# choyingw/SynergyNet

Hardware: NVIDIA H100
Metric: faces/sec (120x120, batch 1024 per GPU, backbone + 3DMM params + 68 landmarks) (higher is better)
Workload: dtype f32

## Files before the change

### synergynet_b200/csrc/kernels_fused.cuh

```cuda
#pragma once
#include "common.cuh"
#include "tc_common.cuh"

namespace syn {

constexpr int kFusedWorkerWarps = 8;
static_assert(kFusedWorkerWarps % 4 == 0, "worker warps form whole warpgroups");

__host__ __device__ constexpr int ceil_div_c(int a, int b) { return (a + b - 1) / b; }
__host__ __device__ constexpr int round_up_c(int a, int b) { return ceil_div_c(a, b) * b; }

template <int CIN_, int CHID_, int NC_, int COUT_, int W_, int STRIDE_, int RO_, int FACES_, bool RES_, int WSTREAM_>
struct FusedCfg {
  static constexpr bool RES = RES_;
  static constexpr bool WSTREAM = WSTREAM_ > 0;
  static constexpr int CIN = CIN_;
  static constexpr int CIN_P = round_up_c(CIN_, 16);
  static constexpr int CHID = CHID_, NC = NC_, NCHUNK = CHID_ / NC_;
  static constexpr int COUT = COUT_, COUT_P = round_up_c(COUT_, 16);
  static constexpr int W = W_, STRIDE = STRIDE_, WO = (W_ - 1) / STRIDE_ + 1;
  static constexpr int RO = RO_, STRIPS = WO / RO_, FACES = FACES_;
  static constexpr int RWIN = (RO_ - 1) * STRIDE_ + 3;
  static constexpr int ROWS_MAX = (RWIN < W_ ? RWIN : W_);
  static constexpr int M1_MAX = FACES_ * ROWS_MAX * W_;
// ... 41 lines not shown
  int* sat;
  int npass;
#ifdef SYN_FUSED_TRACE
  int trace_id;
#endif
};

#ifdef SYN_FUSED_TRACE
__device__ long long g_fused_trace[18 * 2 * 64 * 8];
#define SYN_TRACE(role, chunk, ev)                                                                        \
  do {                                                                                                    \
    if (trace_on) g_fused_trace[((p.trace_id * 2 + (role)) * 64 + (chunk)) * 8 + (ev)] = clock64();      \
  } while (0)
#else
#define SYN_TRACE(role, chunk, ev) do { } while (0)
#endif

template <int THREADS>
__device__ __forceinline__ void group_bar_sync(int grp) {
  switch (grp) {
    case 0: asm volatile("bar.sync 1, %0;" ::"n"(THREADS) : "memory"); break;
    case 1: asm volatile("bar.sync 2, %0;" ::"n"(THREADS) : "memory"); break;
    case 2: asm volatile("bar.sync 3, %0;" ::"n"(THREADS) : "memory"); break;
    default: asm volatile("bar.sync 4, %0;" ::"n"(THREADS) : "memory"); break;
  }
}

__host__ __device__ constexpr int fused_d2_pieces(int cout_p, int slabs, int nwg) {
  int s = 1;
  while (slabs * s < nwg && (cout_p / (2 * s)) % 8 == 0) s *= 2;
  return s;
}

template <int N, int KSTEPS, int NPASS>
__device__ __forceinline__ void fused_mma_group(float* acc, uint32_t d_hi, uint32_t a_lo, uint32_t a_plane, uint32_t a_kstep,
                                                uint32_t b_lo, uint32_t b_plane, uint32_t b_kstep, bool acc_in) {
  tc::wgmma_fence();
#pragma unroll
  for (int pass = 0; pass < NPASS; ++pass)
#pragma unroll
    for (int ks = 0; ks < KSTEPS; ++ks)
      tc::wgmma_f16<N>(acc, tc::desc64(d_hi, a_lo + (((pass == 2 ? a_plane : 0) + ks * a_kstep) >> 4)),
                       tc::desc64(d_hi, b_lo + (((pass == 1 ? b_plane : 0) + ks * b_kstep) >> 4)),
                       (acc_in || pass > 0 || ks > 0) ? 1u : 0u);
  tc::wgmma_commit();
}

template <class C>
__global__ void __launch_bounds__((kFusedWorkerWarps + 1) * 32, 1) fused_mbconv_kernel(const FusedArgs p) {
  constexpr int NWW = kFusedWorkerWarps;
  constexpr int NWT = NWW * 32;
  constexpr int NWG = NWW / 4;
  constexpr int NKG_ = C::NC / 8;
  constexpr int NG = 1;
  constexpr int WPG = NWW / NG, TPG = WPG * 32;
  constexpr int KPG = NKG_ / NG;
  constexpr int NSPL = fused_d2_pieces(C::COUT_P, C::SLABS2, NWG);
  constexpr int N2 = C::COUT_P / NSPL;
  constexpr int IPW = ceil_div_c(C::SLABS2 * NSPL, NWG);
  static_assert(N2 % 8 == 0 && N2 <= 256, "MMA N");
  using namespace tc;
  extern __shared__ __align__(1024) uint8_t smem_raw[];
  __shared__ __align__(8) uint64_t bar_w, bar_wfull[4], bar_wempty[4];

  uint8_t* smem = smem_raw + ((1024u - (smem_u32(smem_raw) & 1023u)) & 1023u);
  const int tid = threadIdx.x, warp = tid >> 5;
// ... 196 lines not shown
        SYN_TRACE(0, c, 3);
      };
      {
        SYN_TRACE(0, 0, 0);
        const uint8_t* w0 = chunk_slot(g, 0);
        group_bar_sync<TPG>(grp);
        SYN_TRACE(0, 0, 1);
        if constexpr (C::STRIPS > 1) {
          constexpr int CQ = KPG * 2;
          if (iy0 < 0)
            for (int i = gtid; i < C::HS_COLS * CQ; i += TPG)
              *reinterpret_cast<float4*>(sH + (size_t)(i / CQ) * C::HS_STRIDE + grp * KPG * 8 + (i % CQ) * 4) =
                  make_float4(0.f, 0.f, 0.f, 0.f);
          if (iy0 + C::RWIN - 1 > C::W - 1)
            for (int i = gtid; i < C::HS_COLS * CQ; i += TPG)
              *reinterpret_cast<float4*>(sH + (size_t)((C::RWIN - 1) * C::HS_COLS + i / CQ) * C::HS_STRIDE +
                                         grp * KPG * 8 + (i % CQ) * 4) = make_float4(0.f, 0.f, 0.f, 0.f);
        }
        issue_g1(wg < slabs1, acc1[0], wg, w0);
        gemm1_epi1(0, w0);
      }
      for (int c = 0; c < C::NCHUNK; ++c, ++g) {
        const int slot = C::WSTREAM ? (int)(g % C::WSTAGES) : c;
        const uint8_t* wch = sWch + slot * C::CHUNK_BYTES;
        const float* dwc = reinterpret_cast<const float*>(wch + C::CH_DW);
        group_bar_sync<TPG>(grp);
        SYN_TRACE(0, c, 4);
        const bool more = c + 1 < C::NCHUNK;
        const uint8_t* wn = wch;
        if constexpr (!LATE_G1) {
          if (more) wn = chunk_slot(g + 1, c + 1);
          issue_g1(more && wg < slabs1, acc1[0], wg, wn);
        }
        if constexpr (C::STRIDE == 1 && ((C::WO >= 15 && C::WO <= 30) || C::WO == 8)) {
          constexpr int XL = (C::WO >= 15) ? 8 : 4, YL = 8 / XL;
          constexpr int CPR = (C::WO + 1) / 2, XG2 = (CPR + XL - 1) / XL, RP2 = (C::RO + 1) / 2;
          constexpr int RPU = (RP2 + YL - 1) / YL, UPK = RPU * XG2;
          const int l8 = tid & 7, qh = (tid >> 3) & 1;
          const int lx = l8 % XL, ly = l8 / XL;
          const bool mir = (l8 & 4) != 0;
          const int units = KPG * nfaces * UPK;
          for (int u = gtid >> 4; u < units; u += TPG / 16) {
            const int kgl = u / (nfaces * UPK), r1 = u - kgl * (nfaces * UPK);
            const int f = r1 / UPK, r2 = r1 - f * UPK;
            const int rpu = r2 / XG2, xg = r2 - rpu * XG2;
            const int kg = grp * KPG + kgl, j0 = kg * 8 + qh * 4;
            const int ox = 2 * (xg * XL + lx), oy = 2 * (rpu * YL + ly);
            if (ox >= C::WO || oy >= C::RO) continue;
            const bool two = (oy + 1 < C::RO);
            const float* wq = dwc + j0;
            float2 w[3][3][2];
#pragma unroll
            for (int ky = 0; ky < 3; ++ky)
#pragma unroll
              for (int kl = 0; kl < 3; ++kl) {
                const float4 t4 = *reinterpret_cast<const float4*>(wq + (ky * 3 + (mir ? 2 - kl : kl)) * C::DWS);
                w[ky][kl][0] = make_float2(t4.x, t4.y); w[ky][kl][1] = make_float2(t4.z, t4.w);
              }
            float2 acc[2][2][2];
            {
              const float4 b4 = *reinterpret_cast<const float4*>(wq + 9 * C::DWS);
#pragma unroll
              for (int ro = 0; ro < 2; ++ro)
#pragma unroll
                for (int a = 0; a < 2; ++a) { acc[ro][a][0] = make_float2(b4.x, b4.y); acc[ro][a][1] = make_float2(b4.z, b4.w); }
            }
            const float* hb = sH + (size_t)(f * C::HS_FACE + oy * C::HS_COLS + ox + (mir ? 3 : 0)) * C::HS_STRIDE + j0;
// ... 220 lines not shown
        bulk_g2s(smem_u32(smem + C::S_B3), p.wimg, C::B3_BYTES, smem_u32(&bar_w));
        for (uint32_t k = 0; k < (uint32_t)C::WSTAGES; ++k)
          if (total_chunks > k) load_chunk(k);
      } else {
        mbar_expect_tx(smem_u32(&bar_w), C::W_BYTES);
        bulk_g2s(smem_u32(smem + C::S_B3), p.wimg, C::W_BYTES, smem_u32(&bar_w));
      }
    }
    __syncwarp();
    if constexpr (C::WSTREAM) {
      for (uint32_t gi = C::WSTAGES; gi < total_chunks; ++gi) {
        mbar_wait(smem_u32(&bar_wempty[gi % C::WSTAGES]), (gi / C::WSTAGES - 1) & 1, p.err);
        if (elect_one()) load_chunk(gi);
        __syncwarp();
      }
    }
  }
}

template <class C>
inline void fused_tile_plan(int batch, int sms, int& split, int& face_groups) {
  if constexpr (C::FACES == 2) {
    const int full = batch / 2, odd = batch & 1, rem = full % sms;
    split = (2 * rem + odd <= sms) ? full - rem : full;
    face_groups = split + (batch - 2 * split);
  } else {
    split = 0;
    face_groups = (batch + C::FACES - 1) / C::FACES;
  }
}

using FusedB2 = FusedCfg<16, 96, 32, 24, 60, 2, 6, 1, false, 0>;
using FusedB3 = FusedCfg<24, 144, 48, 24, 30, 1, 6, 1, true, 0>;
using FusedB4 = FusedCfg<24, 144, 16, 32, 30, 2, 5, 1, false, 0>;
using FusedB56 = FusedCfg<32, 192, 64, 32, 15, 1, 5, 1, true, 0>;
using FusedB7 = FusedCfg<32, 192, 64, 64, 15, 2, 8, 1, false, 0>;
using FusedB8 = FusedCfg<64, 384, 64, 64, 8, 1, 8, 2, true, 3>;
using FusedB11 = FusedCfg<64, 384, 64, 96, 8, 1, 8, 2, false, 2>;
using FusedB12 = FusedCfg<96, 576, 32, 96, 8, 1, 8, 2, true, 3>;
using FusedB14 = FusedCfg<96, 576, 32, 160, 8, 2, 4, 2, false, 3>;
using FusedB15 = FusedCfg<160, 960, 32, 160, 4, 1, 4, 4, true, 3>;
using FusedB17 = FusedCfg<160, 960, 32, 320, 4, 1, 4, 4, false, 2>;

}
```

### synergynet_b200/csrc/synergy_b200.cu

```cuda
#include <math.h>
#include <stdlib.h>
#include <string.h>

#include <algorithm>
#include <new>
#include <vector>

#include "common.cuh"
#include "kernels_simt.cuh"
#include "kernels_tc.cuh"
#include "kernels_fused.cuh"
#include "kernels_stem.cuh"
#include "kernels_tail.cuh"
#include "kernels_dense.cuh"
#include "kernels_gemm.cuh"
#include "kernels_loss.cuh"
#include "kernels_resnet.cuh"
#include "kernels_mbv1.cuh"

using namespace syn;

namespace {

struct HostConv {
  std::vector<float> w, g, b, m, v;
  float eps = 1e-5f;
  bool set = false;
};

struct DevConv {
  float* w = nullptr;
  float* bias = nullptr;
};

}

struct syn_heads;
void syn_heads_destroy(syn_heads* s);
struct syn_resnet;
void syn_resnet_destroy(syn_resnet* s);
struct syn_mbv1;
void syn_mbv1_destroy(syn_mbv1* s);

struct syn_handle {
  int device = 0;
// ... 141 lines not shown
  const ConvDesc& c = plan().conv[layer];
  TcPointwiseArgs a;
  a.A = A; a.Wimg = h->d_tcw + h->tc_off[layer]; a.bias = h->dconv[layer].bias; a.oscale = h->d_tc_oscale + h->tc_osc_off[layer]; a.residual = residual;
  a.out = out; a.M = M; a.K = c.cin; a.N = c.cout; a.Kp = h->tc_kp[layer]; a.nr = h->tc_nr[layer];
  a.relu6 = c.relu6; a.err = h->d_err; a.sat = h->d_sat;
  dim3 grid((M + 127) / 128, h->tc_nranges[layer]);
  tc_pointwise_kernel<<<grid, kTcThreads, kTcSmemBytes, st>>>(a);
  SYN_LAUNCH_CHECK("tc_pointwise_kernel");
  mark(h, st, "tc_pointwise_kernel");
  return SYN_OK;
}

int launch_pointwise(syn_handle* h, const float* A, int layer, const float* residual, float* out,
                     int M, cudaStream_t st) {
  const ConvDesc& c = plan().conv[layer];
  if (h->engine != SYN_ENGINE_SIMT_FP32) return launch_pointwise_tc(h, A, layer, residual, out, M, st);
  return launch_pointwise_simt(h, A, h->dconv[layer], residual, out, M, c.cin, c.cout, c.relu6, st);
}

int launch_depthwise(syn_handle* h, const float* x, int layer, float* y, int batch, cudaStream_t st) {
  const ConvDesc& c = plan().conv[layer];
  const size_t total = (size_t)batch * c.h_out * c.h_out * (c.cout / 4);
  const unsigned grid = (unsigned)((total + 255) / 256);
  depthwise3x3_kernel<<<grid, 256, 0, st>>>(x, h->dconv[layer].w, h->dconv[layer].bias, y, batch,
                                           c.cout, c.h_in, c.h_out, c.stride);
  SYN_LAUNCH_CHECK("depthwise3x3_kernel");
  mark(h, st, "depthwise3x3_kernel");
  return SYN_OK;
}

template <class C>
int launch_fused(syn_handle* h, const float* x, int block, float* y, int batch, cudaStream_t st);
int launch_stem(syn_handle* h, const float* x, const uint8_t* x_u8, float* y, int batch, cudaStream_t st);

int run_backbone(syn_handle* h, const float* x, int batch, float* params, float* pool,
                 int stop_layer, float* dbg_out, cudaStream_t st, const uint8_t* x_u8 = nullptr) {
  const Plan& P = plan();
  int rc = ensure_workspace(h, batch, st);
  if (rc != SYN_OK) return rc;
  if (x_u8 != nullptr && !h->fused()) {
    if (batch > h->x_f32_batch) {
      if ((rc = refuse_capture(st, "batch %d: the uint8 crops' fp32 scratch (%d faces)" SYN_EAGER_FIRST, batch, h->x_f32_batch))) return rc;
      SYN_CUDA(cudaDeviceSynchronize());
      cudaFree(h->d_x_f32);
      h->d_x_f32 = nullptr;
      h->x_f32_batch = 0;
      SYN_CUDA(grow_alloc(&h->d_x_f32, (size_t)batch * 3 * kImg * kImg * sizeof(float), h->fill_on_grow));
      h->x_f32_batch = batch;
    }
    const size_t n4 = (size_t)batch * 3 * kImg * kImg / 4;
    normalize_u8_kernel<<<(unsigned)((n4 + 255) / 256), 256, 0, st>>>(x_u8, h->d_x_f32, n4, h->center_crop);
    SYN_LAUNCH_CHECK("normalize_u8_kernel");
    mark(h, st, "normalize_u8_kernel");
    x = h->d_x_f32;
    x_u8 = nullptr;
  }

  auto dbg = [&](int layer, const float* buf) -> int {
    const ConvDesc& c = P.conv[layer];
    const size_t n = (size_t)batch * c.h_out * c.h_out * c.cout;
    SYN_CUDA(cudaMemcpyAsync(dbg_out, buf, n * sizeof(float), cudaMemcpyDeviceToDevice, st));
    return SYN_OK;
  };

  int cur = 0;
  int li = 1;
  if (h->fused()) {
    if (stop_layer >= 0 && stop_layer <= 50 && (stop_layer < 2 || (stop_layer - 2) % 3 != 0))
      return fail(SYN_ERR_UNSUPPORTED, "conv %d lives inside a fused block and is never materialised", stop_layer);
    const float* in = x;
    for (int b = 1; b <= 17; ++b) {
      float* out = h->buf_io[cur ^ 1];
      switch (b) {
        case 1: rc = launch_stem(h, in, x_u8, out, batch, st); break;
        case 2: rc = launch_fused<FusedB2>(h, in, b, out, batch, st); break;
        case 3: rc = launch_fused<FusedB3>(h, in, b, out, batch, st); break;
        case 4: rc = launch_fused<FusedB4>(h, in, b, out, batch, st); break;
        case 5: case 6: rc = launch_fused<FusedB56>(h, in, b, out, batch, st); break;
        case 7: rc = launch_fused<FusedB7>(h, in, b, out, batch, st); break;
        case 8: case 9: case 10: rc = launch_fused<FusedB8>(h, in, b, out, batch, st); break;
        case 11: rc = launch_fused<FusedB11>(h, in, b, out, batch, st); break;
        case 12: case 13: rc = launch_fused<FusedB12>(h, in, b, out, batch, st); break;
        case 14: rc = launch_fused<FusedB14>(h, in, b, out, batch, st); break;
        case 15: case 16: rc = launch_fused<FusedB15>(h, in, b, out, batch, st); break;
        default: rc = launch_fused<FusedB17>(h, in, b, out, batch, st); break;
      }
      if (rc != SYN_OK) return rc;
      cur ^= 1;
      in = h->buf_io[cur];
      if (stop_layer == 3 * b - 1) return dbg(3 * b - 1, h->buf_io[cur]);
    }
    if (stop_layer == 51)
      return fail(SYN_ERR_UNSUPPORTED, "conv 51 is fused with the average pool and never materialised");
    {
      float* pooled = pool ? pool : h->d_pool_tmp;
      TailArgs t;
      t.x = h->buf_io[cur]; t.wimg = h->d_tail_w; t.bias = h->dconv[51].bias; t.oscale = h->d_tail_osc;
      t.pooled = pooled; t.batch = batch; t.err = h->d_err; t.sat = h->d_sat; t.npass = h->npass();
      const int ntiles = (batch + kTailFaces - 1) / kTailFaces;
      t.ctas_per_slice = std::max(1, std::min(ntiles, h->sm_count / 10));
      tail_conv_pool_kernel<<<10 * t.ctas_per_slice, kTailThreads, kTailSmem, st>>>(t);
      SYN_LAUNCH_CHECK("tail_conv_pool_kernel");
      mark(h, st, "tail_conv_pool_kernel");
      heads_kernel<<<dim3((batch + 7) / 8, 2), 256, 0, st>>>(pooled, h->d_head_w, h->d_head_b, params, batch);
      SYN_LAUNCH_CHECK("heads_kernel");
      mark(h, st, "heads_kernel");
      return SYN_OK;
    }
  } else {
  stem_conv3x3s2_kernel<<<batch * 60, kStemThreads, 0, st>>>(x, h->dconv[0].w, h->dconv[0].bias,
// ... 201 lines not shown
    *reinterpret_cast<uint16_t*>(img.data() + byte_off + plane_bytes) = l;
  };
  float* b3p = reinterpret_cast<float*>(img.data());
  std::vector<float> s3(C::COUT);
  for (int n = 0; n < C::COUT; ++n) {
    s3[n] = channel_scale(w3 + n, (size_t)C::COUT, C::CHID);
    b3p[n] = b3[n];
    b3p[C::COUT_P + n] = 1.0f / (kActScaleHost * s3[n]);
  }
  std::vector<float> s1(C::CHID);
  for (int ch = 0; ch < C::CHID; ++ch) s1[ch] = channel_scale(w1 + ch, (size_t)C::CHID, K);
  for (int c = 0; c < C::NCHUNK; ++c) {
    const size_t chunk = C::B3_BYTES + (size_t)c * C::CHUNK_BYTES;
    float* d = reinterpret_cast<float*>(img.data() + chunk + C::CH_DW);
    for (int n = 0; n < C::NC; ++n) {
      const int ch = c * C::NC + n;
      for (int k = 0; k < K; ++k) {
        const size_t off = (size_t)(n / 8) * 128 + (size_t)(k / 8) * ((C::NC / 8) * 128) + (n % 8) * 16 + (k % 8) * 2;
        put(chunk + C::CH_W1 + off, w1[(size_t)k * C::CHID + ch] * s1[ch], C::W1_PLANE);
      }
      for (int t = 0; t < 9; ++t) d[t * C::DWS + n] = dw[(size_t)t * C::CHID + ch];
      d[9 * C::DWS + n] = bdw[ch] / 6.0f;
      d[10 * C::DWS + 2 * (n & ~1) + (n & 1)] = b1[ch] / 6.0f;
      d[10 * C::DWS + 2 * (n & ~1) + 2 + (n & 1)] = 1.0f / (6.0f * kActScaleHost * s1[ch]);
    }
    for (int n = 0; n < C::COUT; ++n)
      for (int k = 0; k < C::NC; ++k) {
        const size_t off = (size_t)(n / 8) * 128 + (size_t)(k / 8) * ((C::COUT_P / 8) * 128) + (n % 8) * 16 + (k % 8) * 2;
        put(chunk + C::CH_W3 + off, w3[(size_t)(c * C::NC + k) * C::COUT + n] * s3[n], C::W3_PLANE);
      }
  }
}

template <class C>
int launch_fused(syn_handle* h, const float* x, int block, float* y, int batch, cudaStream_t st) {
  static bool attr_set[16] = {};
  if (!attr_set[h->device & 15]) {
    SYN_CUDA(cudaFuncSetAttribute(fused_mbconv_kernel<C>, cudaFuncAttributeMaxDynamicSharedMemorySize, C::SMEM_BYTES));
    attr_set[h->device & 15] = true;
  }
  FusedArgs a;
  a.x = x; a.wimg = h->d_fused + h->fused_off[block]; a.y = y; a.batch = batch; a.err = h->d_err; a.sat = h->d_sat; a.npass = h->npass();
#ifdef SYN_FUSED_TRACE
  a.trace_id = block;
#endif
  fused_tile_plan<C>(batch, h->sm_count, a.split, a.face_groups);
  const int ntiles = a.face_groups * C::STRIPS;
  cudaLaunchConfig_t cfg = {};
  cfg.gridDim = dim3(std::min(ntiles, h->sm_count));
  cfg.blockDim = dim3((kFusedWorkerWarps + 1) * 32);
  cfg.dynamicSmemBytes = C::SMEM_BYTES;
  cfg.stream = st;
  cudaLaunchAttribute attr[1];
  attr[0].id = cudaLaunchAttributeProgrammaticStreamSerialization;
  attr[0].val.programmaticStreamSerializationAllowed = 1;
  cfg.attrs = attr;
  cfg.numAttrs = 1;
  SYN_CUDA(cudaLaunchKernelEx(&cfg, fused_mbconv_kernel<C>, a));
  SYN_LAUNCH_CHECK("fused_mbconv_kernel");
  static const char* const names[18] = {"", "", "fused_block2", "fused_block3", "fused_block4",
                                        "fused_block5", "fused_block6", "fused_block7", "fused_block8", "fused_block9",
                                        "fused_block10", "fused_block11", "fused_block12", "fused_block13", "fused_block14",
                                        "fused_block15", "fused_block16", "fused_block17"};
  mark(h, st, names[block]);
  return SYN_OK;
}

int launch_stem(syn_handle* h, const float* x, const uint8_t* x_u8, float* y, int batch, cudaStream_t st) {
  using C = StemCfg;
  static bool attr_set[16] = {};
  if (!attr_set[h->device & 15]) {
    SYN_CUDA(cudaFuncSetAttribute(stem_block1_kernel, cudaFuncAttributeMaxDynamicSharedMemorySize, C::SMEM_BYTES));
    attr_set[h->device & 15] = true;
  }
  StemArgs a;
  a.x = x; a.x_u8 = x_u8; a.wimg = h->d_fused + h->fused_off[1]; a.y = y; a.ntiles = batch * C::STRIPS;
  a.err = h->d_err; a.sat = h->d_sat; a.border = x_u8 != nullptr ? h->center_crop : 0; a.npass = h->npass();
  cudaLaunchConfig_t cfg = {};
  cfg.gridDim = dim3(std::min((a.ntiles + 1) / 2, h->sm_count));
  cfg.blockDim = dim3(kStemB1Threads);
  cfg.dynamicSmemBytes = C::SMEM_BYTES;
  cfg.stream = st;
  cudaLaunchAttribute attr[1];
  attr[0].id = cudaLaunchAttributeProgrammaticStreamSerialization;
  attr[0].val.programmaticStreamSerializationAllowed = 1;
  cfg.attrs = attr;
  cfg.numAttrs = 1;
  SYN_CUDA(cudaLaunchKernelEx(&cfg, stem_block1_kernel, a));
  SYN_LAUNCH_CHECK("stem_block1_kernel");
  mark(h, st, "fused_stem_block1");
  return SYN_OK;
}

void pack_recon_tc(std::vector<uint8_t>& img, std::vector<float>& meta, const std::vector<float>& planar, int64_t n,
                   int64_t pad, const float* ascale) {
  const int64_t vtiles = pad / 128;
  img.assign((size_t)vtiles * kDnATile, 0);
// ... 251 lines not shown
      all.insert(all.end(), img.begin(), img.end());
      all.resize((all.size() + 1023) / 1024 * 1024);
    }
    if (h->d_tcw) { cudaFree(h->d_tcw); h->d_tcw = nullptr; }
    SYN_CUDA(cudaMalloc(&h->d_tcw, all.size()));
    SYN_CUDA(cudaMemcpy(h->d_tcw, all.data(), all.size(), cudaMemcpyHostToDevice));
    int rc_o = upload(&h->d_tc_oscale, osc_all);
    if (rc_o != SYN_OK) return rc_o;
    if (h->d_err == nullptr) {
      SYN_CUDA(cudaHostAlloc(&h->d_err, sizeof(int), cudaHostAllocMapped | cudaHostAllocPortable));
      SYN_CUDA(cudaMalloc(&h->d_sat, sizeof(int)));
    }
    *reinterpret_cast<volatile int*>(h->d_err) = 0;
    SYN_CUDA(cudaMemset(h->d_sat, 0, sizeof(int)));
    SYN_CUDA(cudaFuncSetAttribute(tc_pointwise_kernel, cudaFuncAttributeMaxDynamicSharedMemorySize, kTcSmemBytes));
    h->tc_ready = true;
  }
  {
    std::vector<uint8_t> all, img;
    auto W = [&](int l) { return slab.data() + w_off[l]; };
    auto Bv = [&](int l) { return slab.data() + b_off[l]; };
    auto add = [&](int block) {
      h->fused_off[block] = all.size();
      all.insert(all.end(), img.begin(), img.end());
      all.resize((all.size() + 1023) / 1024 * 1024);
    };
    pack_fused<StemCfg>(img, W(0), Bv(0), W(1), Bv(1), W(2), Bv(2)); add(1);
    auto blk = [&](int b, auto tag) {
      using Cfg = decltype(tag);
      const int e = 3 * b - 3;
      pack_fused<Cfg>(img, W(e), Bv(e), W(e + 1), Bv(e + 1), W(e + 2), Bv(e + 2));
      add(b);
    };
    blk(2, FusedB2{}); blk(3, FusedB3{}); blk(4, FusedB4{}); blk(5, FusedB56{}); blk(6, FusedB56{});
    blk(7, FusedB7{}); blk(8, FusedB8{}); blk(9, FusedB8{}); blk(10, FusedB8{}); blk(11, FusedB11{});
    blk(12, FusedB12{}); blk(13, FusedB12{}); blk(14, FusedB14{}); blk(15, FusedB15{}); blk(16, FusedB15{});
    blk(17, FusedB17{});
    {
      const float* w = W(51);
      std::vector<uint8_t> timg((size_t)10 * kTailWBytes, 0);
      std::vector<float> tosc(kTailN);
      for (int n = 0; n < kTailN; ++n) {
        const float sc = channel_scale(w + n, (size_t)kTailN, kTailK);
        tosc[n] = 1.0f / (kActScaleHost * sc);
        const int slice = n / 128, r = n % 128;
        for (int k = 0; k < kTailK; ++k) {
          const int kc = k / kTailKC, kl = k % kTailKC;
          const size_t off = (size_t)slice * kTailWBytes + (size_t)kc * 2 * kTailPlane + (size_t)(r / 8) * 128 +
                             (size_t)(kl / 8) * 2048 + (r % 8) * 16 + (kl % 8) * 2;
          uint16_t hi, lo;
          split_f16_host(w[(size_t)k * kTailN + n] * sc, hi, lo);
          *reinterpret_cast<uint16_t*>(timg.data() + off) = hi;
          *reinterpret_cast<uint16_t*>(timg.data() + off + kTailPlane) = lo;
        }
      }
      if (h->d_tail_w) { cudaFree(h->d_tail_w); h->d_tail_w = nullptr; }
      SYN_CUDA(cudaMalloc(&h->d_tail_w, timg.size()));
      SYN_CUDA(cudaMemcpy(h->d_tail_w, timg.data(), timg.size(), cudaMemcpyHostToDevice));
      int rc_t = upload(&h->d_tail_osc, tosc);
      if (rc_t != SYN_OK) return rc_t;
      SYN_CUDA(cudaFuncSetAttribute(tail_conv_pool_kernel, cudaFuncAttributeMaxDynamicSharedMemorySize, kTailSmem));
    }
    if (h->d_fused) { cudaFree(h->d_fused); h->d_fused = nullptr; }
    SYN_CUDA(cudaMalloc(&h->d_fused, all.size()));
    SYN_CUDA(cudaMemcpy(h->d_fused, all.data(), all.size(), cudaMemcpyHostToDevice));
  }
  int rc;
// ... 390 lines not shown
```

Baseline: 269,300.

## Add dual-pipeline large MBConv kernel for block 4 with independent warpgroup tiles

Replaces the generic fused MBConv kernel for block 4 with a new kernel where two worker warpgroups each run their own strip pipeline, with private input, activation and hidden buffers and shared weights loaded once by a producer warp. Each warpgroup converts the next tile's input to split fp16 after finishing the current one and prefetches the tile after that into L2. The intent is to overlap two independent tiles' GEMM, depthwise and epilogue phases so tensor cores and ALUs stay busy. It costs more shared memory per CTA and keeps one CTA per SM, and the grid is sized to half the tile count.

```diff
diff --git a/synergynet_b200/csrc/kernels_fused.cuh b/synergynet_b200/csrc/kernels_fused.cuh
--- a/synergynet_b200/csrc/kernels_fused.cuh
+++ b/synergynet_b200/csrc/kernels_fused.cuh
@@ -646,7 +646,6 @@
 
 using FusedB2 = FusedCfg<16, 96, 32, 24, 60, 2, 6, 1, false, 0>;
 using FusedB3 = FusedCfg<24, 144, 48, 24, 30, 1, 6, 1, true, 0>;
-using FusedB4 = FusedCfg<24, 144, 16, 32, 30, 2, 5, 1, false, 0>;
 using FusedB56 = FusedCfg<32, 192, 64, 32, 15, 1, 5, 1, true, 0>;
 using FusedB7 = FusedCfg<32, 192, 64, 64, 15, 2, 8, 1, false, 0>;
 using FusedB8 = FusedCfg<64, 384, 64, 64, 8, 1, 8, 2, true, 3>;
diff --git a/synergynet_b200/csrc/kernels_large.cuh b/synergynet_b200/csrc/kernels_large.cuh
--- /dev/null
+++ b/synergynet_b200/csrc/kernels_large.cuh
@@ -0,0 +1,363 @@
+#pragma once
+#include "common.cuh"
+#include "tc_common.cuh"
+#include "kernels_fused.cuh"
+
+namespace syn {
+
+template <int CIN_, int CHID_, int NC_, int COUT_, int W_, int STRIDE_, int RO_, bool RES_>
+struct LargeCfg : FusedCfg<CIN_, CHID_, NC_, COUT_, W_, STRIDE_, RO_, 1, RES_, 0> {
+  using F = FusedCfg<CIN_, CHID_, NC_, COUT_, W_, STRIDE_, RO_, 1, RES_, 0>;
+  static constexpr int A2_TILE = 64 * NC_ * 2, A2_PLANE = F::SLABS2 * A2_TILE;
+  static constexpr int H_BYTES = F::RWIN * F::HS_COLS * F::HS_STRIDE * 4;
+  static constexpr int P_XA = 0, P_A2 = P_XA + 2 * F::XA_PLANE, P_H = P_A2 + 2 * A2_PLANE;
+  static constexpr int PIPE_BYTES = round_up_c(P_H + H_BYTES, 1024);
+  static constexpr int S_PIPE = round_up_c(F::W_BYTES, 1024);
+  static constexpr int SMEM_BYTES = S_PIPE + 2 * PIPE_BYTES + 1024;
+  static_assert(SMEM_BYTES <= 227 * 1024, "shared memory");
+  static_assert(F::COUT_P <= 256 && F::COUT_P % 8 == 0, "GEMM2 N: one column piece");
+};
+
+using LargeB4 = LargeCfg<24, 144, 16, 32, 30, 2, 5, false>;
+
+#ifdef SYN_FUSED_TRACE
+#define LARGE_TRACE(row, ev)                                                                                   \
+  do {                                                                                                        \
+    if (trace_on) g_fused_trace[((p.trace_id * 2 + pl) * 64 + (row)) * 8 + (ev)] = clock64();                \
+  } while (0)
+#else
+#define LARGE_TRACE(row, ev) do { } while (0)
+#endif
+
+constexpr int kLargeThreads = 9 * 32;
+
+template <class C>
+__global__ void __launch_bounds__(kLargeThreads, 1) large_mbconv_kernel(const FusedArgs p) {
+  using namespace tc;
+  constexpr int PT = 128;
+  constexpr int NWW = 8;
+  constexpr int NKG = C::NC / 8;
+  extern __shared__ __align__(1024) uint8_t smem_raw[];
+  __shared__ __align__(8) uint64_t bar_w;
+
+  uint8_t* smem = smem_raw + ((1024u - (smem_u32(smem_raw) & 1023u)) & 1023u);
+  const int tid = threadIdx.x, warp = tid >> 5;
+  const int ntiles = p.batch * C::STRIPS;
+  const int step = 2 * (int)gridDim.x;
+
+  asm volatile("griddepcontrol.launch_dependents;" ::: "memory");
+  if (tid == 0) {
+    mbar_init(smem_u32(&bar_w), 1);
+    fence_mbar_init();
+  }
+  __syncthreads();
+
+  const uint8_t* sWch = smem + C::B3_BYTES;
+  const float* sB3 = reinterpret_cast<const float*>(smem);
+
+  if (warp < NWW) {
+    const int pl = __shfl_sync(0xffffffffu, warp >> 2, 0);
+    const int ptid = tid - pl * PT;
+    uint8_t* pbase = smem + C::S_PIPE + pl * C::PIPE_BYTES;
+    uint8_t* sXA = pbase + C::P_XA;
+    uint8_t* sA2 = pbase + C::P_A2;
+    float* sH = reinterpret_cast<float*>(pbase + C::P_H);
+    auto pipe_bar = [&]() { group_bar_sync<PT>(pl); };
+
+    for (int i = ptid; i < C::H_BYTES / 16; i += PT) reinterpret_cast<float4*>(sH)[i] = make_float4(0.f, 0.f, 0.f, 0.f);
+    mbar_wait_inl(smem_u32(&bar_w), 0, p.err);
+    const uint32_t d_hi = smem_desc_hi(128);
+    constexpr uint32_t LBO_W1 = (C::NC / 8) * 128, LBO_W3 = (C::COUT_P / 8) * 128;
+
+    auto issue_g1 = [&](bool on, float* acc, int s1, const uint8_t* wch) {
+      if (on) {
+        const uint32_t a_lo = smem_desc_lo(smem_u32(sXA + s1 * C::XA_TILE), 1024);
+        const uint32_t w_lo = smem_desc_lo(smem_u32(wch + C::CH_W1), LBO_W1);
+        if (p.npass == 1) fused_mma_group<C::NC, C::CIN_P / 16, 1>(acc, d_hi, a_lo, C::XA_PLANE, 2048, w_lo, C::W1_PLANE, 2 * LBO_W1, false);
+        else fused_mma_group<C::NC, C::CIN_P / 16, 3>(acc, d_hi, a_lo, C::XA_PLANE, 2048, w_lo, C::W1_PLANE, 2 * LBO_W1, false);
+      } else {
+        wgmma_fence();
+        wgmma_commit();
+      }
+    };
+
+#ifdef SYN_FUSED_TRACE
+    int k_strip = 0;
+#endif
+    auto prep = [&](int tile) {
+      const int f0 = tile / C::STRIPS, sp = tile - f0 * C::STRIPS;
+      const int iy0 = sp * C::RO * C::STRIDE - 1;
+      const int rf = max(iy0, 0), rl = min(iy0 + C::RWIN - 1, C::W - 1);
+      const int M1 = (rl - rf + 1) * C::W;
+#ifdef SYN_FUSED_TRACE
+      const bool trace_on = blockIdx.x == 0 && k_strip == 1 && ptid == 0;
+#endif
+      LARGE_TRACE(62, 0);
+      constexpr int KG = C::CIN_P / 8;
+      constexpr int NXG = PT / 64;
+      constexpr int ITERS = (C::SLABS1 * KG + NXG - 1) / NXG;
+      constexpr int PB = ITERS < 4 ? ITERS : 4;
+      const int r64 = ptid & 63, xg = ptid >> 6;
+      const int n_items = ((M1 + 63) >> 6) * KG;
+      const float* xbase = p.x + ((size_t)(f0 * C::W + rf) * C::W) * C::CIN;
+      for (int e0 = xg; e0 < n_items; e0 += PB * NXG) {
+        float4 qa[PB], qb[PB];
+        bool ok[PB];
+#pragma unroll
+        for (int u = 0; u < PB; ++u) {
+          const int e = min(e0 + u * NXG, n_items - 1);
+          const int t = e / KG, kg = e - t * KG;
+          const int m = t * 64 + r64;
+          ok[u] = (e0 + u * NXG < n_items) && (m < M1) && (kg * 8 < C::CIN);
+          const float* src = xbase + (size_t)min(m, M1 - 1) * C::CIN + min(kg, (C::CIN - 1) / 8) * 8;
+          qa[u] = __ldg(reinterpret_cast<const float4*>(src));
+          qb[u] = __ldg(reinterpret_cast<const float4*>(src + 4));
+        }
+#pragma unroll
+        for (int u = 0; u < PB; ++u) {
+          const int e = e0 + u * NXG;
+          if (e < n_items) {
+            const int t = e / KG, kg = e - t * KG;
+            const float v[8] = {ok[u] ? qa[u].x : 0.f, ok[u] ? qa[u].y : 0.f, ok[u] ? qa[u].z : 0.f, ok[u] ? qa[u].w : 0.f,
+                                ok[u] ? qb[u].x : 0.f, ok[u] ? qb[u].y : 0.f, ok[u] ? qb[u].z : 0.f, ok[u] ? qb[u].w : 0.f};
+            uint32_t h[4], l[4];
+            bool out_of_range = false;
+#pragma unroll
+            for (int j = 0; j < 8; ++j) out_of_range |= act_clamped(v[j]);
+            if (out_of_range) *p.sat = 1;
+#pragma unroll
+            for (int j = 0; j < 4; ++j) split2_f16(v[2 * j] * kActScale, v[2 * j + 1] * kActScale, h[j], l[j]);
+            uint8_t* xa = sXA + t * C::XA_TILE + (r64 >> 3) * 128 + kg * 1024 + (r64 & 7) * 16;
+            *reinterpret_cast<uint4*>(xa) = make_uint4(h[0], h[1], h[2], h[3]);
+            *reinterpret_cast<uint4*>(xa + C::XA_PLANE) = make_uint4(l[0], l[1], l[2], l[3]);
+          }
+        }
+      }
+      LARGE_TRACE(62, 3);
+      fence_proxy_async_smem();
+    };
+    auto prefetch_x = [&](int tile) {
+      if (tile >= ntiles) return;
+      const int f0 = tile / C::STRIPS, sp = tile - f0 * C::STRIPS;
+      const int iy0 = sp * C::RO * C::STRIDE - 1;
+      const int rf = max(iy0, 0), rl = min(iy0 + C::RWIN - 1, C::W - 1);
+      const char* base = reinterpret_cast<const char*>(p.x + ((size_t)(f0 * C::W + rf) * C::W) * C::CIN);
+      const int bytes = (rl - rf + 1) * C::W * C::CIN * 4;
+      for (int o = ptid * 128; o < bytes; o += PT * 128) asm volatile("prefetch.global.L2 [%0];" ::"l"(base + o));
+    };
+
+    asm volatile("griddepcontrol.wait;" ::: "memory");
+    const int first = (int)blockIdx.x + pl * (int)gridDim.x;
+    if (first < ntiles) prep(first);
+    prefetch_x(first + step);
+
+    for (int tile = first; tile < ntiles; tile += step) {
+      const int f0 = tile / C::STRIPS, sp = tile - f0 * C::STRIPS;
+      const int oy0 = sp * C::RO;
+      const int iy0 = oy0 * C::STRIDE - 1;
+      const int rf = max(iy0, 0), rl = min(iy0 + C::RWIN - 1, C::W - 1);
+      const int M1 = (rl - rf + 1) * C::W;
+      const int slabs1 = (M1 + 63) >> 6;
+#ifdef SYN_FUSED_TRACE
+      const bool trace_on = blockIdx.x == 0 && k_strip == 1 && ptid == 0;
+#endif
+      LARGE_TRACE(63, 0);
+      int row = ptid & 127;
+      asm volatile("" : "+r"(row));
+      float acc1[2][C::NC / 2];
+      float acc2[C::SLABS2][C::COUT_P / 2];
+
+      auto gemm1_epi1 = [&](int c) {
+        const uint8_t* wch = sWch + c * C::CHUNK_BYTES;
+        const float* bs1 = reinterpret_cast<const float*>(wch + C::CH_DW) + 10 * C::DWS;
+        float4 bs[C::NC / 8];
+#pragma unroll
+        for (int q = 0; q < C::NC / 8; ++q) bs[q] = *reinterpret_cast<const float4*>(bs1 + 2 * acc_col(row, 4 * q));
+#pragma unroll
+        for (int s1 = 0; s1 < C::SLABS1; ++s1) {
+          if (s1 + 1 < C::SLABS1) issue_g1(s1 + 1 < slabs1, acc1[(s1 + 1) & 1], s1 + 1, wch);
+          if (s1 + 1 < C::SLABS1) wgmma_wait<1>();
+          else wgmma_wait<0>();
+          if (s1 >= slabs1) continue;
+          const float* acc = acc1[s1 & 1];
+#pragma unroll
+          for (int h = 0; h < 2; ++h) {
+            const int m = 64 * s1 + acc_row(row, 2 * h);
+            if (m < M1) {
+              const int yl = m / C::W, xx = m - yl * C::W;
+              float* hrow = sH + (size_t)((rf - iy0 + yl) * C::HS_COLS + xx + 1) * C::HS_STRIDE;
+#pragma unroll
+              for (int q = 0; q < C::NC / 8; ++q) {
+                const int i = 4 * q + 2 * h, j0 = acc_col(row, i);
+                *reinterpret_cast<float2*>(hrow + j0) = make_float2(__saturatef(fmaf(acc[i], bs[q].z, bs[q].x)),
+                                                                   __saturatef(fmaf(acc[i + 1], bs[q].w, bs[q].y)));
+              }
+            }
+          }
+        }
+        wgmma_wait<0>();
+        LARGE_TRACE(c, 3);
+      };
+
+      LARGE_TRACE(0, 0);
+      pipe_bar();
+      LARGE_TRACE(0, 1);
+      if (iy0 < 0)
+        for (int i = ptid; i < C::HS_COLS * (C::NC / 4); i += PT)
+          *reinterpret_cast<float4*>(sH + (size_t)(i / (C::NC / 4)) * C::HS_STRIDE + (i % (C::NC / 4)) * 4) =
+              make_float4(0.f, 0.f, 0.f, 0.f);
+      if (iy0 + C::RWIN - 1 > C::W - 1)
+        for (int i = ptid; i < C::HS_COLS * (C::NC / 4); i += PT)
+          *reinterpret_cast<float4*>(sH + (size_t)((C::RWIN - 1) * C::HS_COLS + i / (C::NC / 4)) * C::HS_STRIDE +
+                                     (i % (C::NC / 4)) * 4) = make_float4(0.f, 0.f, 0.f, 0.f);
+      issue_g1(true, acc1[0], 0, sWch);
+      gemm1_epi1(0);
+      for (int c = 0; c < C::NCHUNK; ++c) {
+        const uint8_t* wch = sWch + c * C::CHUNK_BYTES;
+        const float* dwc = reinterpret_cast<const float*>(wch + C::CH_DW);
+        pipe_bar();
+        LARGE_TRACE(c, 4);
+        const bool more = c + 1 < C::NCHUNK;
+        issue_g1(more, acc1[0], 0, wch + C::CHUNK_BYTES);
+        {
+          constexpr int GX = 8, XG = (C::WO + GX - 1) / GX;
+          constexpr int RP = (C::RO + 1) / 2;
+          constexpr int ITEMS = NKG * XG * RP, QW = PT / 8;
+          constexpr int NR = C::STRIDE + 3;
+          const int lx = ptid & 7;
+          const bool swz = (C::STRIDE == 2) && (lx & 4);
+          const int q0 = swz ? 4 : 0, q1 = 4 - q0;
+#pragma unroll 1
+          for (int it = ptid >> 3; it < ITEMS; it += QW) {
+            const int kg = it % NKG;
+            float2 w[3][3][4];
+            {
+              const float* wbase = dwc + kg * 8;
+#pragma unroll
+              for (int dx = 0; dx < 3; ++dx)
+#pragma unroll
+                for (int dy = 0; dy < 3; ++dy) {
+                  const float4 ta = *reinterpret_cast<const float4*>(wbase + (dy * 3 + dx) * C::DWS + q0);
+                  const float4 te = *reinterpret_cast<const float4*>(wbase + (dy * 3 + dx) * C::DWS + q1);
+                  w[dx][dy][0] = make_float2(ta.x, ta.y); w[dx][dy][1] = make_float2(ta.z, ta.w);
+                  w[dx][dy][2] = make_float2(te.x, te.y); w[dx][dy][3] = make_float2(te.z, te.w);
+                }
+            }
+            const int r2 = it / NKG;
+            const int rp = r2 / XG, xg = r2 - rp * XG;
+            const int ox = xg * GX + lx, oy = 2 * rp;
+            if (ox >= C::WO) continue;
+            const bool two = oy + 1 < C::RO;
+            const float* h0 = sH + (size_t)((oy * C::STRIDE) * C::HS_COLS + ox * C::STRIDE) * C::HS_STRIDE + kg * 8;
+            float2 acc0[4], acc1d[4];
+            {
+              const float4 a = *reinterpret_cast<const float4*>(dwc + kg * 8 + 9 * C::DWS + q0);
+              const float4 e = *reinterpret_cast<const float4*>(dwc + kg * 8 + 9 * C::DWS + q1);
+              acc0[0] = make_float2(a.x, a.y); acc0[1] = make_float2(a.z, a.w); acc0[2] = make_float2(e.x, e.y); acc0[3] = make_float2(e.z, e.w);
+            }
+#pragma unroll
+            for (int j = 0; j < 4; ++j) acc1d[j] = acc0[j];
+#pragma unroll
+            for (int dx = 0; dx < 3; ++dx) {
+#pragma unroll
+              for (int wr = 0; wr < NR; ++wr) {
+                if (wr >= 3 && !two) continue;
+                const float* hp = h0 + (wr * C::HS_COLS + dx) * C::HS_STRIDE;
+                const float4 a = *reinterpret_cast<const float4*>(hp + q0);
+                const float4 e = *reinterpret_cast<const float4*>(hp + q1);
+                const float2 d[4] = {make_float2(a.x, a.y), make_float2(a.z, a.w), make_float2(e.x, e.y), make_float2(e.z, e.w)};
+                if (wr < 3) {
+#pragma unroll
+                  for (int j = 0; j < 4; ++j) acc0[j] = ffma2(d[j], w[dx][wr][j], acc0[j]);
+                }
+                if (wr >= C::STRIDE) {
+#pragma unroll
+                  for (int j = 0; j < 4; ++j) acc1d[j] = ffma2(d[j], w[dx][wr - C::STRIDE][j], acc1d[j]);
+                }
+              }
+            }
+            constexpr float kOut = 6.0f * kActScale;
+#pragma unroll
+            for (int ro = 0; ro < 2; ++ro) {
+              if (ro == 1 && !two) continue;
+              const float2* acc = ro ? acc1d : acc0;
+              const int m2 = (oy + ro) * C::WO + ox;
+              uint32_t h[4], l[4];
+#pragma unroll
+              for (int j = 0; j < 4; ++j)
+                split2_f16<false>(__saturatef(acc[j].x) * kOut, __saturatef(acc[j].y) * kOut, h[j], l[j]);
+              uint8_t* dst = sA2 + (m2 >> 6) * C::A2_TILE + ((m2 & 63) >> 3) * 128 + kg * 1024 + (m2 & 7) * 16;
+              *reinterpret_cast<uint4*>(dst) = swz ? make_uint4(h[2], h[3], h[0], h[1]) : make_uint4(h[0], h[1], h[2], h[3]);
+              *reinterpret_cast<uint4*>(dst + C::A2_PLANE) = swz ? make_uint4(l[2], l[3], l[0], l[1]) : make_uint4(l[0], l[1], l[2], l[3]);
+            }
+          }
+        }
+        LARGE_TRACE(c, 5);
+        fence_proxy_async_smem();
+        pipe_bar();
+        {
+          const uint32_t w_lo = smem_desc_lo(smem_u32(wch + C::CH_W3), LBO_W3);
+#pragma unroll
+          for (int s2 = 0; s2 < C::SLABS2; ++s2) {
+            const uint32_t a_lo = smem_desc_lo(smem_u32(sA2 + s2 * C::A2_TILE), 1024);
+            if (p.npass == 1) fused_mma_group<C::COUT_P, C::NC / 16, 1>(acc2[s2], d_hi, a_lo, C::A2_PLANE, 2048, w_lo, C::W3_PLANE, 2 * LBO_W3, c > 0);
+            else fused_mma_group<C::COUT_P, C::NC / 16, 3>(acc2[s2], d_hi, a_lo, C::A2_PLANE, 2048, w_lo, C::W3_PLANE, 2 * LBO_W3, c > 0);
+          }
+          wgmma_wait<0>();
+        }
+        LARGE_TRACE(c, 6);
+        if (more) {
+          LARGE_TRACE(c + 1, 0);
+          LARGE_TRACE(c + 1, 1);
+          gemm1_epi1(c + 1);
+        }
+      }
+      LARGE_TRACE(63, 1);
+      if (tile + step < ntiles) prep(tile + step);
+      prefetch_x(tile + 2 * step);
+      LARGE_TRACE(63, 2);
+      float* ybase = p.y + ((size_t)(f0 * C::WO + oy0) * C::WO) * C::COUT;
+      const float* xbase = p.x + ((size_t)(f0 * C::W + oy0) * C::W) * C::CIN;
+#pragma unroll
+      for (int s2 = 0; s2 < C::SLABS2; ++s2) {
+#pragma unroll
+        for (int h = 0; h < 2; ++h) {
+          const int pix = 64 * s2 + acc_row(row, 2 * h);
+          if (pix >= C::M2F) continue;
+          float* orow = ybase + (size_t)pix * C::COUT;
+          float2 res[C::COUT_P / 8];
+          if constexpr (C::RES) {
+#pragma unroll
+            for (int q = 0; q < C::COUT_P / 8; ++q) {
+              const int j = acc_col(row, 4 * q);
+              res[q] = j < C::COUT ? __ldg(reinterpret_cast<const float2*>(xbase + (size_t)pix * C::CIN + j)) : make_float2(0.f, 0.f);
+            }
+          }
+#pragma unroll
+          for (int q = 0; q < C::COUT_P / 8; ++q) {
+            const int i = 4 * q + 2 * h, j = acc_col(row, i);
+            if (j < C::COUT) {
+              const float2 bb = *reinterpret_cast<const float2*>(sB3 + j);
+              const float2 sc = *reinterpret_cast<const float2*>(sB3 + C::COUT_P + j);
+              float2 o = make_float2(fmaf(acc2[s2][i], sc.x, bb.x), fmaf(acc2[s2][i + 1], sc.y, bb.y));
+              if constexpr (C::RES) { o.x += res[q].x; o.y += res[q].y; }
+              *reinterpret_cast<float2*>(orow + j) = o;
+            }
+          }
+        }
+      }
+      LARGE_TRACE(63, 4);
+#ifdef SYN_FUSED_TRACE
+      ++k_strip;
+#endif
+    }
+  } else if (warp == NWW) {
+    if (elect_one()) {
+      mbar_expect_tx(smem_u32(&bar_w), C::W_BYTES);
+      bulk_g2s(smem_u32(smem), p.wimg, C::W_BYTES, smem_u32(&bar_w));
+    }
+    __syncwarp();
+  }
+}
+
+}
diff --git a/synergynet_b200/csrc/synergy_b200.cu b/synergynet_b200/csrc/synergy_b200.cu
--- a/synergynet_b200/csrc/synergy_b200.cu
+++ b/synergynet_b200/csrc/synergy_b200.cu
@@ -11,6 +11,7 @@
 #include "kernels_tc.cuh"
 #include "kernels_fused.cuh"
 #include "kernels_stem.cuh"
+#include "kernels_large.cuh"
 #include "kernels_tail.cuh"
 #include "kernels_dense.cuh"
 #include "kernels_gemm.cuh"
@@ -218,6 +219,8 @@
 template <class C>
 int launch_fused(syn_handle* h, const float* x, int block, float* y, int batch, cudaStream_t st);
 int launch_stem(syn_handle* h, const float* x, const uint8_t* x_u8, float* y, int batch, cudaStream_t st);
+template <class C>
+int launch_large(syn_handle* h, const float* x, int block, float* y, int batch, cudaStream_t st);
 
 int run_backbone(syn_handle* h, const float* x, int batch, float* params, float* pool,
                  int stop_layer, float* dbg_out, cudaStream_t st, const uint8_t* x_u8 = nullptr) {
@@ -261,7 +264,7 @@
         case 1: rc = launch_stem(h, in, x_u8, out, batch, st); break;
         case 2: rc = launch_fused<FusedB2>(h, in, b, out, batch, st); break;
         case 3: rc = launch_fused<FusedB3>(h, in, b, out, batch, st); break;
-        case 4: rc = launch_fused<FusedB4>(h, in, b, out, batch, st); break;
+        case 4: rc = launch_large<LargeB4>(h, in, b, out, batch, st); break;
         case 5: case 6: rc = launch_fused<FusedB56>(h, in, b, out, batch, st); break;
         case 7: rc = launch_fused<FusedB7>(h, in, b, out, batch, st); break;
         case 8: case 9: case 10: rc = launch_fused<FusedB8>(h, in, b, out, batch, st); break;
@@ -529,6 +532,11 @@
   }
 }
 
+static const char* const kFusedNames[18] = {"", "", "fused_block2", "fused_block3", "fused_block4",
+                                            "fused_block5", "fused_block6", "fused_block7", "fused_block8", "fused_block9",
+                                            "fused_block10", "fused_block11", "fused_block12", "fused_block13", "fused_block14",
+                                            "fused_block15", "fused_block16", "fused_block17"};
+
 template <class C>
 int launch_fused(syn_handle* h, const float* x, int block, float* y, int batch, cudaStream_t st) {
   static bool attr_set[16] = {};
@@ -555,11 +563,37 @@
   cfg.numAttrs = 1;
   SYN_CUDA(cudaLaunchKernelEx(&cfg, fused_mbconv_kernel<C>, a));
   SYN_LAUNCH_CHECK("fused_mbconv_kernel");
-  static const char* const names[18] = {"", "", "fused_block2", "fused_block3", "fused_block4",
-                                        "fused_block5", "fused_block6", "fused_block7", "fused_block8", "fused_block9",
-                                        "fused_block10", "fused_block11", "fused_block12", "fused_block13", "fused_block14",
-                                        "fused_block15", "fused_block16", "fused_block17"};
-  mark(h, st, names[block]);
+  mark(h, st, kFusedNames[block]);
+  return SYN_OK;
+}
+
+template <class C>
+int launch_large(syn_handle* h, const float* x, int block, float* y, int batch, cudaStream_t st) {
+  static bool attr_set[16] = {};
+  if (!attr_set[h->device & 15]) {
+    SYN_CUDA(cudaFuncSetAttribute(large_mbconv_kernel<C>, cudaFuncAttributeMaxDynamicSharedMemorySize, C::SMEM_BYTES));
+    attr_set[h->device & 15] = true;
+  }
+  FusedArgs a = {};
+  a.x = x; a.wimg = h->d_fused + h->fused_off[block]; a.y = y; a.batch = batch; a.face_groups = batch;
+  a.err = h->d_err; a.sat = h->d_sat; a.npass = h->npass();
+#ifdef SYN_FUSED_TRACE
+  a.trace_id = block;
+#endif
+  const int ntiles = batch * C::STRIPS;
+  cudaLaunchConfig_t cfg = {};
+  cfg.gridDim = dim3(std::min((ntiles + 1) / 2, h->sm_count));
+  cfg.blockDim = dim3(kLargeThreads);
+  cfg.dynamicSmemBytes = C::SMEM_BYTES;
+  cfg.stream = st;
+  cudaLaunchAttribute attr[1];
+  attr[0].id = cudaLaunchAttributeProgrammaticStreamSerialization;
+  attr[0].val.programmaticStreamSerializationAllowed = 1;
+  cfg.attrs = attr;
+  cfg.numAttrs = 1;
+  SYN_CUDA(cudaLaunchKernelEx(&cfg, large_mbconv_kernel<C>, a));
+  SYN_LAUNCH_CHECK("large_mbconv_kernel");
+  mark(h, st, kFusedNames[block]);
   return SYN_OK;
 }
 
@@ -877,7 +911,7 @@
       pack_fused<Cfg>(img, W(e), Bv(e), W(e + 1), Bv(e + 1), W(e + 2), Bv(e + 2));
       add(b);
     };
-    blk(2, FusedB2{}); blk(3, FusedB3{}); blk(4, FusedB4{}); blk(5, FusedB56{}); blk(6, FusedB56{});
+    blk(2, FusedB2{}); blk(3, FusedB3{}); blk(4, LargeB4{}); blk(5, FusedB56{}); blk(6, FusedB56{});
     blk(7, FusedB7{}); blk(8, FusedB8{}); blk(9, FusedB8{}); blk(10, FusedB8{}); blk(11, FusedB11{});
     blk(12, FusedB12{}); blk(13, FusedB12{}); blk(14, FusedB14{}); blk(15, FusedB15{}); blk(16, FusedB15{});
     blk(17, FusedB17{});
```

New measurement: 278,300 (median of 6 runs). 1.03x the previous value.

## Add quad-channel depthwise plan for stride-2 fused MBConv blocks

Applied to the files above, without the earlier changes.

Adds a dedicated depthwise-conv path for stride-2 layers with output width at least 15. Each thread owns a fixed group of four channels, keeps its 3x3 weights and bias in registers for the whole chunk, and computes two output rows per slot so the overlapping input row is reused. Results are written directly into the split-f16 GEMM2 A tile. The aim is to cut shared-memory weight reloads and repeated input reads compared with the generic fallback, at the cost of more registers and possibly uneven slot coverage when the output width is padded to a multiple of 8.

```diff
diff --git a/synergynet_b200/csrc/kernels_fused.cuh b/synergynet_b200/csrc/kernels_fused.cuh
--- a/synergynet_b200/csrc/kernels_fused.cuh
+++ b/synergynet_b200/csrc/kernels_fused.cuh
@@ -97,6 +97,20 @@
   return s;
 }
 
+struct DwQuadPlan {
+  int quad;
+  int slot0;
+  int stride;
+  int wop;
+};
+__host__ __device__ constexpr DwQuadPlan fused_dw_quad_plan(int nc, int wo, int nwt, int t) {
+  const int tpo = nwt / (nc / 8);
+  const int o = t / tpo, r = t - o * tpo;
+  return {2 * o + ((r >> 2) & 1), (r >> 3) * 4 + (r & 3), tpo / 2, round_up_c(wo, 8)};
+}
+template <class C>
+constexpr bool fused_dw_quad_plan_on = C::STRIDE == 2 && C::WO >= 15;
+
 template <int N, int KSTEPS, int NPASS>
 __device__ __forceinline__ void fused_mma_group(float* acc, uint32_t d_hi, uint32_t a_lo, uint32_t a_plane, uint32_t a_kstep,
                                                 uint32_t b_lo, uint32_t b_plane, uint32_t b_kstep, bool acc_in) {
@@ -359,7 +373,65 @@
           if (more) wn = chunk_slot(g + 1, c + 1);
           issue_g1(more && wg < slabs1, acc1[0], wg, wn);
         }
-        if constexpr (C::STRIDE == 1 && ((C::WO >= 15 && C::WO <= 30) || C::WO == 8)) {
+        if constexpr (fused_dw_quad_plan_on<C>) {
+          static_assert(C::FACES == 1, "strip tiles");
+          constexpr int TPQ = NWT / (C::NC / 8) / 2;
+          constexpr int WOP = round_up_c(C::WO, 8), NSLOT = ((C::RO + 1) / 2) * WOP;
+          static_assert(NWT % (C::NC / 8) == 0 && TPQ % 8 == 0, "quarter-warps of the depthwise plan");
+          const DwQuadPlan pl = fused_dw_quad_plan(C::NC, C::WO, NWT, tid);
+          const float* wq = dwc + 4 * pl.quad;
+          float2 w[3][3][2];
+#pragma unroll
+          for (int dx = 0; dx < 3; ++dx)
+#pragma unroll
+            for (int dy = 0; dy < 3; ++dy) {
+              const float4 t4 = *reinterpret_cast<const float4*>(wq + (dy * 3 + dx) * C::DWS);
+              w[dx][dy][0] = make_float2(t4.x, t4.y); w[dx][dy][1] = make_float2(t4.z, t4.w);
+            }
+          const float4 b4 = *reinterpret_cast<const float4*>(wq + 9 * C::DWS);
+#pragma unroll 1
+          for (int k = 0; k < ceil_div_c(NSLOT, TPQ); ++k) {
+            const int s = pl.slot0 + k * TPQ;
+            const int rp = s / WOP, ox = s - rp * WOP;
+            if (s >= NSLOT || ox >= C::WO) continue;
+            const int oy = 2 * rp;
+            const bool two = oy + 1 < C::RO;
+            const float* h0 = sH + (size_t)((oy * C::STRIDE) * C::HS_COLS + ox * C::STRIDE) * C::HS_STRIDE + 4 * pl.quad;
+            float2 acc0[2] = {make_float2(b4.x, b4.y), make_float2(b4.z, b4.w)};
+            float2 acc1[2] = {acc0[0], acc0[1]};
+#pragma unroll
+            for (int dx = 0; dx < 3; ++dx) {
+#pragma unroll
+              for (int wr = 0; wr < C::STRIDE + 3; ++wr) {
+                if (wr >= 3 && !two) continue;
+                const float4 t4 = *reinterpret_cast<const float4*>(h0 + (wr * C::HS_COLS + dx) * C::HS_STRIDE);
+                const float2 d[2] = {make_float2(t4.x, t4.y), make_float2(t4.z, t4.w)};
+                if (wr < 3) {
+#pragma unroll
+                  for (int j = 0; j < 2; ++j) acc0[j] = ffma2(d[j], w[dx][wr][j], acc0[j]);
+                }
+                if (wr >= C::STRIDE) {
+#pragma unroll
+                  for (int j = 0; j < 2; ++j) acc1[j] = ffma2(d[j], w[dx][wr - C::STRIDE][j], acc1[j]);
+                }
+              }
+            }
+            constexpr float kOut = 6.0f * kActScale;
+#pragma unroll
+            for (int ro = 0; ro < 2; ++ro) {
+              if (ro == 1 && !two) continue;
+              const float2 a0 = ro ? acc1[0] : acc0[0], a1 = ro ? acc1[1] : acc0[1];
+              const int m2 = (oy + ro) * C::WO + ox;
+              uint32_t h0s, l0s, h1s, l1s;
+              split2_f16<false>(__saturatef(a0.x) * kOut, __saturatef(a0.y) * kOut, h0s, l0s);
+              split2_f16<false>(__saturatef(a1.x) * kOut, __saturatef(a1.y) * kOut, h1s, l1s);
+              uint8_t* dst = sA2 + (m2 >> 7) * (128 * C::NC * 2) + ((m2 & 127) >> 3) * 128 + (pl.quad >> 1) * 2048 +
+                             (m2 & 7) * 16 + (pl.quad & 1) * 8;
+              *reinterpret_cast<uint2*>(dst) = make_uint2(h0s, h1s);
+              *reinterpret_cast<uint2*>(dst + C::A2_PLANE) = make_uint2(l0s, l1s);
+            }
+          }
+        } else if constexpr (C::STRIDE == 1 && ((C::WO >= 15 && C::WO <= 30) || C::WO == 8)) {
           constexpr int XL = (C::WO >= 15) ? 8 : 4, YL = 8 / XL;
           constexpr int CPR = (C::WO + 1) / 2, XG2 = (CPR + XL - 1) / XL, RP2 = (C::RO + 1) / 2;
           constexpr int RPU = (RP2 + YL - 1) / YL, UPK = RPU * XG2;
```

After: 266,400 before, 276,300 after (median of 6 runs). 3.7% higher.
